# DamRsn/VocoderProject

Measured on AMD Instinct MI355X. Metric: STFT-geometry frames/sec (1024-pt frames, hop 256) through the pitch-corrector/vocoder path, higher is better.
Workload: dtype f64

## Files before the change

### vocoderproject_amd/csrc/vp_common.h

```cpp
#pragma once
#include <stddef.h>

#define VP_MARKS 64
#define VP_ORDER_MAX 100
#define VP_ORDER_MAX_SYNTH 30
#define VP_NOTES_STRIDE 89

struct VpGeom {
    int S, N, F, H, C, cpf, W, h, toKeep, latency, inSize, outSize, tauMax;
    int eLen;
    int orderPitch;
    int tau0;
    int bufferIdxMax;
    int xsSteps;
    int htabGlobal;
    double fs, delta, yinTol;
    double gateThrSum;
    double levEps;
    double eeFloor;
};

struct VpCall {
    int inCounter, outCounter, currCounter;
    int vStart, nWin;
// ... 54 lines not shown
    unsigned int *fault;
    int spinLimit;
    const int *streamMap;
};

#if defined(__HIPCC__)
#define VP_HD __host__ __device__
#else
#define VP_HD
#endif

VP_HD static inline int vp_dy_len(int tauMax) { const int need = 2 * VP_MARKS + (5 * VP_MARKS + 1) / 2; return tauMax + 1 > need ? tauMax + 1 : need; }
VP_HD static inline int vp_cum_len(int tauMax) { return tauMax + 1 > 448 ? tauMax + 1 : 448; }

VP_HD static inline size_t vp_pitch_lds_bytes(const VpGeom &g)
{
    size_t dbl = (size_t)(g.toKeep + g.F) + 12 + (size_t)(g.xsSteps - 1) * g.C + g.eLen + 2 * (size_t)g.F + (size_t)vp_dy_len(g.tauMax) + (size_t)vp_cum_len(g.tauMax) + 2 * (VP_ORDER_MAX + 1) + (2 * (size_t)g.tauMax + 4) + (g.htabGlobal ? 0 : 2 * (size_t)g.tauMax + 2);
    return dbl * sizeof(double) + 8 * 16 + sizeof(VpPitchState) + 64 + 64;
}
VP_HD static inline size_t vp_pitch_acc_lds_bytes(const VpGeom &g) { return ((size_t)g.N + g.C + 1 + g.C + 128) * sizeof(double) + 16; }

#define WS_MAXI 24
#define WS_MAXS 8
#define WS_NBG 4
#define WS_ORDER_MAX 24
#define WS_AF(g) ((g).orderPitch > 15 ? 32 : 16)
#define WS_HP(g) ((g).orderPitch > 16 ? 192 : 128)
#define WS_HIST(g) ((g).orderPitch > 15 ? 32 : 16)

struct WsCtl {
    int psDone;
    int fillTurn;
    int bgPub, bgAdopt;
    int prodBar, bgBar;
    int xcDone, zeroDone, pDone, acDone, lpcDone, pickState, pickDone;
    int tDone;
    int pickT[2];
    int iirDone;
    int pubMode;
    int lpcZ[2];
    int instMode[WS_MAXI];
    int ishareBG[4], ishareP[4];
    int fftFlag[4];
    int gNext[WS_MAXS + 1];
    int gDone[WS_MAXI];
    int gNT[WS_MAXS + 1], gLo[WS_MAXS + 1], gHi[WS_MAXS + 1], gNg[WS_MAXS + 1];
};

struct VpWsSched {
    int nInst, nStart, nSeg;
    int instStep[WS_MAXI], instK[WS_MAXI], instPar[WS_MAXI], instStart[WS_MAXI];
    int startStep[WS_MAXS], startPar[WS_MAXS], startNeed[WS_MAXS];
    int segA[WS_MAXS + 1], segB[WS_MAXS + 1];
};
VP_HD static inline bool ws_build_sched(const VpGeom &g, int nChunk0, int nSteps, VpWsSched &sc)
{
    int nCh = nChunk0, par = 0, nI = 0, nS = 0, nG = 0;
    int lastUse[2] = {0, 0};
    for (int t = 0; t < nSteps; t++) {
        if (nCh != 0) {
            if (nI >= WS_MAXI) return false;
            if (nI == 0) { if (nG > WS_MAXS) return false; sc.segA[nG] = 0; sc.segB[nG] = 0; nG++; }
            sc.instStep[nI] = t; sc.instK[nI] = nCh; sc.instPar[nI] = par; sc.instStart[nI] = -1;
            sc.segB[nG - 1] = nI;
            nI++;
            lastUse[par] = nI;
        }
        if (nCh == g.cpf - 1) nCh = 0;
        if (nCh == 0) {
            if (nI >= WS_MAXI || nS >= WS_MAXS || nG > WS_MAXS) return false;
            par ^= 1;
            sc.instStep[nI] = t; sc.instK[nI] = 0; sc.instPar[nI] = par; sc.instStart[nI] = nS;
            sc.startStep[nS] = t; sc.startPar[nS] = par; sc.startNeed[nS] = lastUse[par];
            sc.segA[nG] = nI; sc.segB[nG] = nI; nG++;
            nI++; nS++;
            lastUse[par] = nI;
        }
        nCh += 1;
    }
    sc.nInst = nI; sc.nStart = nS; sc.nSeg = nG;
    return nI > 0;
}

#define WS_MB_MAX 16
#define WS_MB_SCHEDS 4
struct VpWsMb {
    int nBlocks;
    int schedOf[WS_MB_MAX], nChunk0[WS_MB_MAX], inCtr[WS_MB_MAX], outCtr[WS_MB_MAX], currCtr[WS_MB_MAX];
    VpWsSched sc[WS_MB_SCHEDS];
};

struct WsCarve {
    int xs, eF, fr, qtab, htab, P, dY, gtab, r, aPrev, hp, aF, xp, hist, tw, oA, st, ctl, end;
};
VP_HD static inline int ws_even(int v) { return (v + 1) & ~1; }
VP_HD static inline WsCarve ws_carve(const VpGeom &g, int nSteps)
{
    WsCarve c;
    int o = 0;
    c.xs = o;    o += ws_even(g.toKeep + g.F + (nSteps - 1) * g.C + 4);
    c.eF = o;    o += ws_even(g.eLen);
    c.fr = o;    o += 4 * g.F + 2048;
    c.qtab = o;  o += ws_even(2 * g.tauMax + 4);
    c.htab = o;  o += ws_even(2 * g.tauMax + 2);
    c.P = o;     o += ws_even(g.F + g.tauMax + 2 > 450 ? g.F + g.tauMax + 2 : 450);
    c.dY = o;    o += ws_even(vp_dy_len(g.tauMax) + 1);
    c.gtab = o;  o += 2 * VP_MARKS + (6 * VP_MARKS + 1) / 2 + 1;
    o = ws_even(o);
    c.r = o;     o += 2 * 64;
    c.aPrev = o; o += 2 * (VP_ORDER_MAX + 1 + 1);
    c.hp = o;    o += 2 * WS_HP(g);
    c.aF = o;    o += 2 * WS_AF(g);
    c.xp = o;    o += (g.orderPitch > 15 ? 128 : 64);
    c.hist = o;  o += 2 * WS_HIST(g);
    c.tw = o;    o += 2 * VP_FFT_TW_D2;
    c.oA = o;    o += ws_even(g.N + g.C + 1);
    c.st = o;    o += 2 * ((int)(sizeof(VpPitchState) + 15) / 16 * 2);
    c.ctl = o;   o += ((int)sizeof(WsCtl) + 7) / 8;
    c.end = ws_even(o);
    return c;
}
VP_HD static inline size_t vp_pitch_ws_lds_bytes(const VpGeom &g, int nSteps) { return (size_t)ws_carve(g, nSteps).end * sizeof(double); }

VP_HD static inline size_t voc_wave_doubles(int W)
{
    return (size_t)4 * W + 2 * (VP_ORDER_MAX + 1) + 2 * (VP_ORDER_MAX_SYNTH + 1) + 2;
}
#define VP_VOC_SHARED_DOUBLES(W) ((size_t)(W) + 20 + 16 + 8)
```

### vocoderproject_amd/csrc/vp_filters.inc

```

__device__ __forceinline__ double bcast_f64(double v, int src)
{
    int lo = __double2loint(v), hi = __double2hiint(v);
    lo = __builtin_amdgcn_readlane(lo, src);
    hi = __builtin_amdgcn_readlane(hi, src);
    return __hiloint2double(hi, lo);
}

template <class RP, class AP>
__device__ __forceinline__ bool levinson_wave(RP r, AP a, int order, int aLen, double eps, lds_f64 *scratch = nullptr)
{
    const int lane = vp_tid() & 63;
    if (fabs(r[0]) < eps) {
        for (int i = lane; i < aLen; i += WAVE) a[i] = (i == 0) ? 1.0 : 0.0;
        return true;
    }
    const double r0 = r[0];
    if (scratch && order < WAVE) {
        typedef double d2 __attribute__((ext_vector_type(2)));
        typedef __attribute__((address_space(3))) d2 lds_d2;
        lds_d2 *pr = (lds_d2 *)scratch;
        double av = 0.0;
        if (lane == 0) av = 1.0;
        if (lane == 1) av = r[1] / r0;
// ... 840 lines not shown
#define VP_BI_ROW(XQ, Q) \
    VP_BI_T(acc0, XQ, H[16 * Q + 0], 0);   VP_BI_T(acc1, XQ, H[16 * Q + 1], 1);   VP_BI_T(acc2, XQ, H[16 * Q + 2], 2);   \
    VP_BI_T(acc3, XQ, H[16 * Q + 3], 3);   VP_BI_T(acc0, XQ, H[16 * Q + 4], 4);   VP_BI_T(acc1, XQ, H[16 * Q + 5], 5);   \
    VP_BI_T(acc2, XQ, H[16 * Q + 6], 6);   VP_BI_T(acc3, XQ, H[16 * Q + 7], 7);   VP_BI_T(acc0, XQ, H[16 * Q + 8], 8);   \
    VP_BI_T(acc1, XQ, H[16 * Q + 9], 9);   VP_BI_T(acc2, XQ, H[16 * Q + 10], 10); VP_BI_T(acc3, XQ, H[16 * Q + 11], 11); \
    VP_BI_T(acc0, XQ, H[16 * Q + 12], 12); VP_BI_T(acc1, XQ, H[16 * Q + 13], 13); VP_BI_T(acc2, XQ, H[16 * Q + 14], 14); \
    VP_BI_T(acc3, XQ, H[16 * Q + 15], 15);
template <bool RAGGED = false>
__device__ __forceinline__ void iir_block_wave_regs(const lds_f64 *x, lds_f64 *y, int n, const lds_f64 *aL, int order_,
                                                    bool haveHist0, const lds_f64 *hpad)
{
    const int lane = vp_tid() & 63, m = lane & 15;
    const int order = __builtin_amdgcn_readfirstlane(order_);
    {
        double H[64];
#pragma unroll
        for (int j = 16; j < 64; j++) H[j] = hpad[WAVE + lane - j];
        for (int b = 0; b < n; b += WAVE) {
            double X1 = x[RAGGED ? min(b + 16 + m, n - 1) : b + 16 + m], X2 = x[RAGGED ? min(b + 32 + m, n - 1) : b + 32 + m], X3 = x[RAGGED ? min(b + 48 + m, n - 1) : b + 48 + m];
            if (RAGGED) { X1 = (b + 16 + m < n) ? X1 : 0.0; X2 = (b + 32 + m < n) ? X2 : 0.0; X3 = (b + 48 + m < n) ? X3 : 0.0; asm volatile("s_nop 1" : "+v"(X1), "+v"(X2), "+v"(X3)); }
            double acc0 = 0.0, acc1 = 0.0, acc2 = 0.0, acc3 = 0.0;
            VP_BI_ROW(X1, 1)
            VP_BI_ROW(X2, 2)
            VP_BI_ROW(X3, 3)
            if (!RAGGED || b + lane < n) y[b + lane] = (acc0 + acc1) + (acc2 + acc3);
        }
    }
    double H[16], A[16];
#pragma unroll
    for (int j = 0; j < 16; j++) H[j] = hpad[WAVE + lane - j];
#pragma unroll
    for (int k = 1; k <= 16; k++) A[k - 1] = (m + k <= order) ? -aL[m + k] : 0.0;
    double X0 = (!RAGGED || m < n) ? x[RAGGED ? min(m, n - 1) : m] : 0.0;
    for (int b = 0; b < n; b += WAVE) {
        const bool hist = (b > 0) || haveHist0;
        double Y3 = 0.0;
        if (hist && 16 - m <= order) Y3 = y[b - 16 + m];
        const double parked = (!RAGGED || b + lane < n) ? y[RAGGED ? min(b + lane, n - 1) : b + lane] : 0.0;
        double u0 = 0.0, u1 = 0.0;
        VP_BI_T(u0, Y3, A[0], 15);  VP_BI_T(u1, Y3, A[1], 14);  VP_BI_T(u0, Y3, A[2], 13);  VP_BI_T(u1, Y3, A[3], 12);
        VP_BI_T(u0, Y3, A[4], 11);  VP_BI_T(u1, Y3, A[5], 10);  VP_BI_T(u0, Y3, A[6], 9);   VP_BI_T(u1, Y3, A[7], 8);
        VP_BI_T(u0, Y3, A[8], 7);   VP_BI_T(u1, Y3, A[9], 6);   VP_BI_T(u0, Y3, A[10], 5);  VP_BI_T(u1, Y3, A[11], 4);
        VP_BI_T(u0, Y3, A[12], 3);  VP_BI_T(u1, Y3, A[13], 2);  VP_BI_T(u0, Y3, A[14], 1);  VP_BI_T(u1, Y3, A[15], 0);
        X0 = X0 + (u0 + u1);
        asm volatile("s_nop 1" : "+v"(X0));
        double acc0 = 0.0, acc1 = 0.0, acc2 = 0.0, acc3 = 0.0;
        VP_BI_ROW(X0, 0)
        if (!RAGGED || b + lane < n) y[b + lane] = parked + ((acc0 + acc1) + (acc2 + acc3));
        const int bn = b + WAVE;
        if (bn < n) X0 = (!RAGGED || bn + m < n) ? x[RAGGED ? min(bn + m, n - 1) : bn + m] : 0.0;
    }
}

__device__ __forceinline__ void iir_hc_phase1(const lds_f64 *x, lds_f64 *y, int n, const lds_f64 *hpad, double gmul)
{
    const int lane = vp_tid() & 63, m = lane & 15;
    {
        double H[64];
#pragma unroll
        for (int j = 0; j < 64; j++) H[j] = hpad[WAVE + lane - j];
        for (int b = 0; b < n; b += WAVE) {
            double X0 = gmul * x[b + m], X1 = gmul * x[b + 16 + m], X2 = gmul * x[b + 32 + m], X3 = gmul * x[b + 48 + m];
            double acc0 = 0.0, acc1 = 0.0, acc2 = 0.0, acc3 = 0.0;
            asm volatile("s_nop 1" : "+v"(X0), "+v"(X1), "+v"(X2), "+v"(X3));
            VP_BI_ROW(X0, 0)
            VP_BI_ROW(X1, 1)
            VP_BI_ROW(X2, 2)
            VP_BI_ROW(X3, 3)
            y[b + lane] = (acc0 + acc1) + (acc2 + acc3);
        }
    }
}
template <int RN = 48>
__device__ __forceinline__ void iir_hc_phase2(lds_f64 *y, int n, const lds_f64 *aL, int order_, int nh0, const lds_f64 *hpad,
                                              int *flag = nullptr, int gen = 0, const VpTmo *timeouts = nullptr)
{
    static_assert(RN == 32 || RN == 48, "32 or 48 history columns");
    const int lane = vp_tid() & 63, m = lane & 15;
    const int order = __builtin_amdgcn_readfirstlane(order_);
    STAMPG_BEGIN();
    double R[RN];
    {
        const lds_f64 *h = hpad + WAVE;
        const double h0 = h[lane + 1], h1 = (lane + 65 < 128) ? h[lane + 65] : 0.0;
        double c0 = h0, c1 = h1;
        R[0] = c0;
        const double areg = (lane + 1 <= order) ? aL[lane + 1] : 0.0;
#pragma unroll
        for (int k = 1; k < RN; k++) {
            const double ak = bcast_f64(areg, k - 1);
            const double up = bcast_f64(c1, 0);
            double n0 = wave_shl1_f64(c0);
            const double n1 = wave_shl1_f64(c1);
            if (lane == 63) n0 = up;
            c0 = __builtin_fma(ak, h0, n0);
            c1 = __builtin_fma(ak, h1, n1);
            R[k] = c0;
        }
    }
    STAMPG(24);
    if (flag) {
        int spin = 0;
        const int lim = timeouts ? timeouts->limit : (1 << 22);
        for (; spin < lim && __hip_atomic_load(flag, __ATOMIC_ACQUIRE, __HIP_MEMORY_SCOPE_WORKGROUP) != gen; spin++)
            __builtin_amdgcn_s_sleep(1);
        if (spin == lim && lane == 0 && timeouts) vp_timeout(*timeouts);
// ... 92 lines not shown
```

### vocoderproject_amd/csrc/vp_pitch_ws.inc

```

#ifdef VP_STAMPS
#define WS_SLOT(D, W, E) (D).dbg[64 + g.S + (c.nChunk0 & 3) * 128 + (W) * 8 + (E)]
#define WS_EV(D, W, E) do { if (blockIdx.x == 0 && (threadIdx.x & 63) == 0) atomicAdd(&WS_SLOT(D, W, E), (unsigned long long)wall_clock64()); } while (0)
#define WS_EV0(D, W, E) do { if (blockIdx.x == 0 && threadIdx.x == 0) atomicAdd(&WS_SLOT(D, W, E), (unsigned long long)wall_clock64()); } while (0)
#define WS_TB() unsigned long long ws_tb_ = wall_clock64()
#define WS_TA(D, W, E) do { if (blockIdx.x == 0 && (threadIdx.x & 63) == 0) { const unsigned long long t_ = wall_clock64(); atomicAdd(&WS_SLOT(D, W, E), t_ - ws_tb_); ws_tb_ = t_; } } while (0)
#define WS_TR() do { ws_tb_ = wall_clock64(); } while (0)
#define WS_FINE(D, K) do { if (i == 0) WS_EV(D, 12 + (K) / 8, (K) % 8); } while (0)
#define WS_FINEP(D, K) do { if (si == 0 && rank < 2) WS_EV(D, 13 + rank, K); } while (0)
#define WS_FINER(D, J) do { if ((J) < 7) WS_EV(D, 15, J); } while (0)
#define WS_STAT(D, K, V) do { if (blockIdx.x == 0 && (threadIdx.x & 63) == 0) atomicAdd(&(D).dbg[64 + g.S + (K)], (unsigned long long)(V)); } while (0)
#define WS_CLK() wall_clock64()
#else
#define WS_EV(D, W, E) do { } while (0)
#define WS_EV0(D, W, E) do { } while (0)
#define WS_TB() do { } while (0)
#define WS_TA(D, W, E) do { } while (0)
#define WS_TR() do { } while (0)
#define WS_FINE(D, K) do { } while (0)
#define WS_FINEP(D, K) do { } while (0)
#define WS_FINER(D, J) do { } while (0)
#define WS_STAT(D, K, V) do { } while (0)
#define WS_CLK() 0ULL
#endif
// ... 30 lines not shown
    double loc = 0.0;
#pragma unroll
    for (int u = 0; u < 24; u++) { const int j = j0 + u; if (u < per && j < nb) loc += v[u] * v[u]; }
    double inc = loc;
    for (int off = 1; off < WAVE; off <<= 1) { const double o = __shfl_up(inc, off, WAVE); if (lane >= off) inc += o; }
    double run = inc - loc;
#pragma unroll
    for (int u = 0; u < 24; u++) { const int j = j0 + u; if (u < per && j <= nb) { P[j] = run; if (j < nb) run += v[u] * v[u]; } }
}

__device__ __forceinline__ void ws_yin_pick_wave(const VpGeom &g, const VpDev &d, const PitchLds &L, lds_state *st)
{
    const int lane = vp_tid() & 63;
    for (int k = 1 + lane; k < g.tauMax; k += WAVE) {
        const double cm = L.cum[k], q = (double)k / cm;
        L.dY[k] = L.dY[k] * q;
    }
    wave_sync();
    int tau = INT_MAX;
    for (int k0 = g.tau0; k0 < g.tauMax; k0 += WAVE) {
        const int k = k0 + lane;
        const unsigned long long m = __ballot(k < g.tauMax && L.dY[min(k, g.tauMax - 1)] < g.yinTol);
        if (m) { tau = k0 + (int)__builtin_ctzll(m); break; }
    }
    if (tau < g.tauMax) {
        while (true) {
            const double a = L.dY[tau + 1], b = L.dY[tau];
            if (!(a < b)) break;
            tau += 1;
            if (tau + 1 >= g.tauMax) break;
        }
        if (lane == 0) {
            if (tau >= g.tauMax) atomicAdd(&d.ub[3], 1ULL);
            st->pitch = g.fs / tau;
            st->period = tau;
        }
    }
}


struct SegTab {
    lds_f64 *x0, *xN;
    lds_i32 *stMark, *srcBase, *flags, *startIdx, *stopIdx, *eLim;
};
__device__ __forceinline__ SegTab ws_seg_tab(lds_f64 *base)
{
    SegTab G;
    G.x0 = base; G.xN = base + VP_MARKS;
    G.stMark = (lds_i32 *)(base + 2 * VP_MARKS); G.srcBase = G.stMark + VP_MARKS; G.flags = G.srcBase + VP_MARKS;
    G.startIdx = G.flags + VP_MARKS; G.stopIdx = G.startIdx + VP_MARKS; G.eLim = G.stopIdx + VP_MARKS;
    return G;
}
__device__ __forceinline__ void ws_psola_table_seg(const VpGeom &g, const VpDev &d, const lds_state *st, lds_state *stIdx, const SegTab &G, int kFirst, int kLast,
                                                   int pSFirst, lds_ctl *ctl, int sg)
{
    const int lane = vp_tid() & 63;
    const int T = (st->pitch > 1) ? st->period : st->prevVoicedPeriod;
    const int nG = 2 * T + 1;
    const int nSt = st->nSt;
    const int smi0 = stIdx->stMarkIdx;
    const int smi = smi0 + lane;
    const bool have = smi < nSt;
    const int stMark = have ? st->stMarks[smi] : 0;
    const int v = stMark - T;
    const int kd = max(kFirst, v >= 0 ? v / g.C : 0);
    const bool due = have && kd <= kLast;
    const unsigned long long notDue = ~__ballot(due);
    const int ng = notDue ? (int)__builtin_ctzll(notDue) : 64;
    if (lane < ng) {
        const int pS = pSFirst + (kd - kFirst) * g.C;
        bool q2 = false;
        int clIdx = closest_an_mark_idx(g, st, stMark, T, kd, pS, q2);
        if (q2) atomicAdd(&d.ub[0], 1ULL);
        int clAnMark;
        if (clIdx >= 0)
            clAnMark = st->anMarks[clIdx];
        else {
            int j = st->nPrevAn - clIdx;
            atomicAdd(&d.ub[1], 1ULL);
            clAnMark = (j >= 0 && j < VP_MARKS) ? st->prevAnMarks[j] : 0;
        }
        const double dSt = (double)stMark;
        const double beta = st->beta;
        const double x0 = dSt + (double)(0 - T) / beta;
        const double xN = dSt + (double)(nG - 1 - T) / beta;
        G.x0[lane] = x0; G.xN[lane] = xN;
        G.stMark[lane] = stMark;
        G.srcBase[lane] = g.toKeep + clAnMark - T;
        G.flags[lane] = (smi == 0 ? 1 : 0) | (smi == nSt - 1 ? 2 : 0);
        G.startIdx[lane] = max(max((int)floor(x0), 0), kd * g.C);
        G.stopIdx[lane] = min((int)ceil(xN), g.F);
        G.eLim[lane] = min(g.eLen, g.toKeep + g.F + kd * g.C);
    }
    int lo = 0, hi = 0;
    if (lane < ng) { lo = G.startIdx[lane]; hi = G.stopIdx[lane]; }
    lo = __builtin_amdgcn_readfirstlane(lo);
#pragma unroll
    for (int off = 32; off > 0; off >>= 1) hi = max(hi, __shfl_xor(hi, off, WAVE));
    if (lane == 0) {
        stIdx->stMarkIdx = smi0 + ng;
        ctl->gNg[sg] = ng; ctl->gLo[sg] = lo; ctl->gHi[sg] = hi;
        ctl->gNT[sg] = (ng > 0 && hi > lo) ? (hi - lo + WAVE - 1) / WAVE : 0;
    }
}
__device__ __forceinline__ void ws_psola_gather_seg(const VpGeom &g, const VpDev &d, const PitchLds &L, const SegTab &G, lds_ctl *ctl, int sg, int jA, int jB,
                                                    int kFirst, bool first)
{
    const lds_state *st = L.st;
    const int lane = vp_tid() & 63;
    const int nT = ctl->gNT[sg], lo = ctl->gLo[sg], hi = ctl->gHi[sg], ng = ctl->gNg[sg];
    const lds_f64 *hw = L.htab;
    bool have = false;
    int T = 0, nG = 1;
    double beta = 1.0, mx0 = 0.0, mxN = 0.0;
    int mst = 0, msrc = 0, mfl = 0, ma = 0, mb = 0, mlim = 0;
    auto below = [&](int x) -> int { return (x <= lo) ? 0 : min((x - lo + WAVE - 1) / WAVE, nT); };
    auto count = [&](int r) -> int {
        const int a = (r == 0) ? 0 : below((kFirst + r) * g.C), b = (r == jB - jA) ? nT : below((kFirst + r + 1) * g.C);
        return b - a;
    };
    auto release = [&](int j) {
        ws_wait_ge(&ctl->psDone, j, d);
        for (;;) {
            if (lane == 0) ctl->instMode[j] = 2;
            ws_signal(&ctl->psDone, j + 1);
            j++;
            if (j > jB || count(j - jA) != 0) break;
        }
    };
    if (first) {
        if (count(0) == 0) release(jA);
    }
    for (;;) {
        int m = 0;
        if (lane == 0) m = __hip_atomic_fetch_add((lds_i32 *)&ctl->gNext[sg], 1, __ATOMIC_RELAXED, __HIP_MEMORY_SCOPE_WORKGROUP);
        m = __builtin_amdgcn_readfirstlane(m);
        if (m >= nT) break;
        const unsigned long long tTrip0 = WS_CLK();
        (void)tTrip0;
        if (!have) {
            have = true;
            T = (st->pitch > 1) ? st->period : st->prevVoicedPeriod;
            nG = 2 * T + 1;
            beta = st->beta;
            const int ql = max(min(lane, ng - 1), 0);
            mx0 = G.x0[ql]; mxN = G.xN[ql];
            mst = G.stMark[ql]; msrc = G.srcBase[ql]; mfl = G.flags[ql]; ma = G.startIdx[ql]; mb = G.stopIdx[ql]; mlim = G.eLim[ql];
        }
        const int b = lo + WAVE * m;
        const int i = b + lane;
        const bool in = i < hi;
        const double di = (double)i;
        double accv = in ? L.oE[i] : 0.0;
        unsigned long long mask = __ballot(lane < ng && ma < b + WAVE && mb > b);
        struct Entry { int sa, sb, stM, srcBase, fl, eLim; double x0, xN; };
        auto entry = [&](int q) -> Entry {
            Entry e;
            e.sa = __builtin_amdgcn_readlane(ma, q); e.sb = __builtin_amdgcn_readlane(mb, q);
            e.x0 = __hiloint2double(__builtin_amdgcn_readlane(__double2hiint(mx0), q), __builtin_amdgcn_readlane(__double2loint(mx0), q));
            e.xN = __hiloint2double(__builtin_amdgcn_readlane(__double2hiint(mxN), q), __builtin_amdgcn_readlane(__double2loint(mxN), q));
            e.stM = __builtin_amdgcn_readlane(mst, q); e.srcBase = __builtin_amdgcn_readlane(msrc, q); e.fl = __builtin_amdgcn_readlane(mfl, q);
            e.eLim = __builtin_amdgcn_readlane(mlim, q);
            return e;
        };
        auto slow = [&](const Entry &e, bool &act) -> double {
            act = in && i >= e.sa && i < e.sb && di >= e.x0 && di <= e.xN;
            if (!act) return 0.0;
            const double dSt = (double)e.stM;
            int j = (int)ceil((di - dSt) * beta) + T;
            j = max(0, min(j, nG - 1));
            const double q0 = L.qtab[j], qm = L.qtab[max(j - 1, 0)], qp = L.qtab[min(j + 1, nG - 1)];
            double xj = dSt + q0, xjm = 0.0;
            if (j < nG - 1 && xj < di) {
                xjm = xj; j++; xj = dSt + qp;
                while (j < nG - 1 && xj < di) { xjm = xj; j++; xj = dSt + L.qtab[j]; }
            } else if (j > 0) {
                xjm = dSt + qm;
// ... 9 lines not shown
                const int src = e.srcBase + jj;
                const double ev = (src >= 0 && src < e.eLim) ? L.eF[src] : 0.0;
                const bool windowed = (e.fl & 1) ? (jj >= T) : ((e.fl & 2) ? (jj < T) : true);
                return windowed ? ev * hw[jj] : ev;
            };
            if (j > 0) {
                const double ya = ys(j - 1), yb = ys(j);
                return ya + (yb - ya) / (xj - xjm) * (di - xjm);
            }
            return ys(0);
        };
        auto fast = [&](const Entry &e, bool &act, bool &ok) -> double {
            act = in && i >= e.sa && i < e.sb && di >= e.x0 && di <= e.xN;
            const double dSt = (double)e.stM;
            int j0 = (int)ceil((di - dSt) * beta) + T;
            j0 = max(0, min(j0, nG - 1));
            const double q0 = L.qtab[j0], qm = L.qtab[max(j0 - 1, 0)], qp = L.qtab[min(j0 + 1, nG - 1)];
            const double xj0 = dSt + q0, xm0 = dSt + qm, xp0 = dSt + qp;
            const bool up = j0 < nG - 1 && xj0 < di;
            const bool upMore = up && (j0 + 1 < nG - 1) && xp0 < di;
            const bool down = !up && j0 > 0 && xm0 >= di;
            ok = !act || !(upMore || down);
            const int j = up ? j0 + 1 : j0;
            const double xj = up ? xp0 : xj0, xjm = up ? xj0 : xm0;
            const int ja = max(j - 1, 0);
            const int srcA = e.srcBase + ja, srcB = e.srcBase + j;
            const double ea = L.eF[max(0, min(srcA, e.eLim - 1))], eb = L.eF[max(0, min(srcB, e.eLim - 1))];
            const double ha = hw[ja], hb = hw[j];
            const double eva = (srcA >= 0 && srcA < e.eLim) ? ea : 0.0, evb = (srcB >= 0 && srcB < e.eLim) ? eb : 0.0;
            const bool wa = (e.fl & 1) ? (ja >= T) : ((e.fl & 2) ? (ja < T) : true), wb = (e.fl & 1) ? (j >= T) : ((e.fl & 2) ? (j < T) : true);
            const double ya = wa ? eva * ha : eva, yb = wb ? evb * hb : evb;
            const double itp = ya + (yb - ya) / (xj - xjm) * (di - xjm);
            return (j > 0) ? itp : yb;
        };
        while (mask) {
            const int q1 = (int)__builtin_ctzll(mask);
            mask &= mask - 1;
            const bool two = mask != 0;
            const int q2 = two ? (int)__builtin_ctzll(mask) : q1;
            mask &= mask - 1;
            const Entry e1 = entry(q1), e2 = entry(q2);
            bool a1, a2, ok1, ok2;
            double v1 = fast(e1, a1, ok1), v2 = fast(e2, a2, ok2);
            WS_STAT(d, 2, 1);
#ifdef WS_GATHER_TEST
            if (WS_GATHER_TEST == 1) ok1 = false;
            if (WS_GATHER_TEST == 2 && ((b >> 6) & 1) && lane == 5) ok2 = false;
#endif
            if (__ballot(!(ok1 && ok2))) { v1 = slow(e1, a1); v2 = slow(e2, a2); WS_STAT(d, 3, 1); }
            if (a1) accv += v1;
            if (two && a2) accv += v2;
        }
        if (in) L.oE[i] = accv;
        WS_STAT(d, 0, 1); WS_STAT(d, 1, WS_CLK() - tTrip0);
        int r = 0;
        for (int q = 1; q <= jB - jA; q++) r += (b >= (kFirst + q) * g.C) ? 1 : 0;
        __threadfence_block();
        int was = 0;
        if (lane == 0) was = __hip_atomic_fetch_add((lds_i32 *)&ctl->gDone[jA + r], 1, __ATOMIC_ACQ_REL, __HIP_MEMORY_SCOPE_WORKGROUP);
        was = __builtin_amdgcn_readfirstlane(was);
        if (was + 1 == count(r)) release(jA + r);
    }
}

template <bool FAST, bool BIG>
__device__ __forceinline__ void ws_background(const VpGeom &g0, const VpCall &c, const VpDev &d, const VpWsSched &sc, lds_f64 *sm, const WsCarve &cv0,
                                              lds_ctl *ctl, int bw, int gateOpen)
{
    lds_state *stBG = (lds_state *)(sm + cv0.st) + 1;
    const bool lead = bw == WS_NBG - 1;
    int bgBarGen = 0;
    PitchLds L;
    L.qtab = nullptr; L.htab = nullptr;
    L.st = stBG;
    L.ishare = (int *)ctl->ishareBG;
    L.fftFlag = (int *)ctl->fftFlag;
    L.xcA = nullptr;
    L.oA = nullptr; L.pend = nullptr;
    L.gateOpen = gateOpen;
    const int wq = (int)(blockDim.x / WAVE) - WS_NBG + bw;
    (void)wq;
    const int nStart = sc.nStart;
    for (int i = 0; i < nStart; i++) {
        const int gen = i + 1;
        VpGeom g = g0;
        WsCarve cv = cv0;
        asm volatile("" : "+s"(g.tauMax), "+s"(g.F), "+s"(g.C), "+s"(g.toKeep), "+s"(g.orderPitch), "+s"(g.tau0));
        asm volatile("" : "+s"(cv.xs), "+s"(cv.fr), "+s"(cv.P), "+s"(cv.dY), "+s"(cv.r), "+s"(cv.aPrev), "+s"(cv.hp), "+s"(cv.xp), "+s"(cv.aF), "+s"(cv.tw));
        L.eF = sm + cv.P;
        L.cum = sm + cv.P;
        L.dY = sm + cv.dY;
        L.fftTw = (lds_d2 *)(sm + cv.tw);
        if (lead) WS_FINE(d, 0);
        const int lane = vp_tid() & 63;
        if (!gateOpen) {
            if (lead) {
                ws_wait_ge(&ctl->bgAdopt, i, d);
                if (lane == 0) { stBG->nAn = 0; stBG->prevPitch = 0; stBG->gateOpen = 0; ctl->pubMode = 0; }
                ws_signal(&ctl->bgPub, gen);
            }
            continue;
        }
        const int pn = sc.startPar[i], tS = sc.startStep[i];
        ws_wait_ge(&ctl->fillTurn, sc.startNeed[i], d);
        if (i == 0) WS_EV(d, wq, 0);
        L.xs = sm + cv.xs + ((g.toKeep - g.tauMax) & 1) + tS * g.C;
// ... 122 lines not shown
            WS_FINE(d, 2);
            pitch_marks(g, L, d.ub);
            WS_FINE(d, 3);
            place_st_marks(g, c, d, stBG, nr, notesN);
        }
        wave_sync();
        if (i == 0) WS_EV(d, wq, 4);
        ws_wait_ge(&ctl->lpcDone, gen, d);
        if (stBG->nAn != 0) {
            const int ncopy = ctl->lpcZ[pn] ? VP_ORDER_MAX + 1 : g.orderPitch + 1;
            for (int q = lane; q < ncopy; q += WAVE) stBG->a[q] = L.aPrev[q];
        }
        WS_FINE(d, 4);
        ws_wait_ge(&ctl->zeroDone, (WS_NBG - 1) * gen, d);
        WS_FINE(d, 5);
        if (lane == 0) ctl->pubMode = stBG->nAn != 0 ? 2 : 1;
        ws_signal(&ctl->bgPub, gen);
        WS_EV(d, wq, i == 0 ? 5 : 6);
        VP_PRIO_DOWN();
    }
}

template <bool FAST>
__device__ __forceinline__ void ws_producer(const VpGeom &g, const VpCall &c, const VpDev &d, const VpWsSched &sc, lds_f64 *sm, const WsCarve &cv,
                                            lds_ctl *ctl, int rank, int nP, int gateOpen, bool firstBlock = true, bool lastBlock = true)
{
    const int lane = vp_tid() & 63, tp = rank * WAVE + lane, ntp = nP * WAVE;
    lds_state *st = (lds_state *)(sm + cv.st), *stPub = st + 1;
    lds_f64 *xsAll = sm + cv.xs + ((g.toKeep - g.tauMax) & 1);
    lds_f64 *frBase = sm + cv.fr;
    int barGen = 0;
    bool qValid = false;
    PitchLds L;
    L.st = st;
    L.eF = sm + cv.eF;
    L.qtab = sm + cv.qtab;
    L.htab = sm + cv.htab;
    const SegTab G = ws_seg_tab(sm + cv.gtab);
    const int order = g.orderPitch;
    const int wq = rank + 2;
    (void)wq;
    WS_EV(d, wq, 0);
    WS_TB();
    const int s_ = vp_stream(d);
    if (firstBlock && c.nChunk0 != 0 && st->nAn != 0) {
        const double *ge = d.eFrame + (size_t)s_ * g.eLen;
        const int lim = min(g.eLen, g.toKeep + g.F + (c.nChunk0 - 1) * g.C);
        for (int q = tp; q < lim; q += ntp) L.eF[q] = ge[q];
    }
    for (int sg = 0; sg < sc.nSeg; sg++) {
        const int jA = sc.segA[sg], jB = sc.segB[sg];
        const int t = sc.instStep[jA], kFirst = sc.instK[jA], kLast = sc.instK[jB], p = sc.instPar[jA], si = sc.instStart[jA];
        const int pS = c.pStart + t * g.C;
        WS_TR();
        L.xs = xsAll + t * g.C;
        L.oE = p ? frBase + 3 * g.F + 2048 : frBase;
        L.yF = p ? frBase + 2 * g.F + 2048 : frBase + g.F;
        int mode;
        if (si >= 0) {
            const int jEnd = g.toKeep + g.F + (jB - jA) * g.C;
            if (gateOpen && rank != 0) {
                ws_wait_ge(&ctl->lpcDone, si + 1, d);
                WS_TA(d, wq, 1);
                const lds_f64 *aN = sm + cv.aF + p * WS_AF(g);
                for (int q = 4 * (tp - WAVE); q < jEnd; q += 4 * (ntp - WAVE)) fir4((const lds_f64 *)L.xs, aN, order, q, jEnd, L.eF);
                for (int q = jEnd + tp - WAVE; q < g.eLen; q += ntp - WAVE) L.eF[q] = 0.0;
                WS_TA(d, wq, 2);
                ws_wait_ge(&ctl->tDone, si + 1, d);
                WS_TA(d, wq, 1);
                const int T = ctl->pickT[p];
                const double *hg = d.hannTab + d.hannOff[T];
                for (int q = tp - WAVE; q < 2 * T + 1; q += ntp - WAVE) L.htab[q] = hg[q];
                WS_TA(d, wq, 2);
            }
            ws_wait_ge(&ctl->bgPub, si + 1, d);
            WS_TA(d, wq, 1);
            WS_FINEP(d, 0);
            mode = ctl->pubMode;
            if (rank == 0) {
                if (mode == 2) {
                    if (lane == 0) st->stMarkIdx = 0;
                    wave_sync();
                    ws_psola_table_seg(g, d, stPub, st, G, kFirst, kLast, pS, ctl, sg);
                }
                WS_TA(d, wq, 4);
                WS_FINEP(d, 2);
            } else {
                if (rank == 1) {
                    const int keep = (int)(offsetof(VpPitchState, stMarkIdx) / sizeof(int));
                    const lds_i32 *src = (const lds_i32 *)stPub;
                    lds_i32 *dst = (lds_i32 *)st;
                    for (int q = lane; q < (int)(sizeof(VpPitchState) / sizeof(int)); q += WAVE) if (q != keep) dst[q] = src[q];
                    WS_FINEP(d, 1);
                }
                if (mode == 2) {
                    const int T = (stPub->pitch > 1) ? stPub->period : stPub->prevVoicedPeriod;
                    const double beta = stPub->beta;
                    for (int q = tp - WAVE; q < 2 * T + 1; q += ntp - WAVE) L.qtab[q] = (double)(q - T) / beta;
                }
                WS_TA(d, wq, 2);
                WS_FINEP(d, 2);
            }
            if (mode == 1) for (int q = tp; q < jEnd; q += ntp) L.eF[q] = 0.0;
            qValid = mode == 2;
            ws_group_barrier(&ctl->prodBar, nP, barGen, d);
            WS_TA(d, wq, 3);
            WS_FINEP(d, 3);
            if (rank == 0) ws_signal(&ctl->bgAdopt, si + 1);
        } else {
            mode = (st->nAn != 0) ? 2 : 0;
            if (mode == 2) {
                if (rank == 0) {
                    ws_psola_table_seg(g, d, st, st, G, kFirst, kLast, pS, ctl, sg);
                    WS_TA(d, wq, 4);
                } else {
                    const int j0 = g.toKeep + g.F - g.C, jEnd = j0 + (jB - jA + 1) * g.C;
                    for (int q = j0 + 4 * (tp - WAVE); q < jEnd; q += 4 * (ntp - WAVE)) fir4((const lds_f64 *)L.xs, (const lds_f64 *)st->a, order, q, jEnd, L.eF + kFirst * g.C);
                    for (int q = kFirst * g.C + jEnd + tp - WAVE; q < g.eLen; q += ntp - WAVE) L.eF[q] = 0.0;
                    if (!qValid) {
                        const int T = (st->pitch > 1) ? st->period : st->prevVoicedPeriod;
                        const double beta = st->beta;
                        const double *hg = d.hannTab + d.hannOff[T];
                        for (int q = tp - WAVE; q < 2 * T + 1; q += ntp - WAVE) { L.qtab[q] = (double)(q - T) / beta; L.htab[q] = hg[q]; }
                    }
                    WS_TA(d, wq, 2);
                }
                qValid = true;
                ws_group_barrier(&ctl->prodBar, nP, barGen, d);
                WS_TA(d, wq, 3);
            }
        }
        if (mode == 2) {
            ws_psola_gather_seg(g, d, L, G, ctl, sg, jA, jB, kFirst, rank == 0);
            WS_FINEP(d, 4);
            WS_TA(d, wq, 5);
            ws_wait_ge(&ctl->psDone, jB + 1, d);
            WS_FINEP(d, 6);
            WS_TA(d, wq, 3);
        } else {
            ws_group_barrier(&ctl->prodBar, nP, barGen, d);
            WS_TA(d, wq, 3);
            if (rank == 0) {
                if (lane <= jB - jA) ctl->instMode[jA + lane] = (lane == 0) ? mode : 0;
                ws_signal(&ctl->psDone, jB + 1);
            }
        }
    }
    {
        int nChunkEnd = c.nChunk0;
        for (int t = 0; t < c.nSteps; t++) { if (nChunkEnd == g.cpf - 1) nChunkEnd = 0; nChunkEnd += 1; }
        if (lastBlock && nChunkEnd != 0 && st->nAn != 0) {
            double *ge = d.eFrame + (size_t)s_ * g.eLen;
            for (int q = tp; q < g.eLen; q += ntp) ge[q] = L.eF[q];
        }
    }
    WS_EV(d, wq, 7);
}

template <bool FAST, bool BIG>
__device__ __forceinline__ void ws_recursion(const VpGeom &g, const VpCall &c, const VpDev &d, const VpWsSched &sc, lds_f64 *sm, const WsCarve &cv,
                                             lds_ctl *ctl, int me, int nIir, double gainPitch)
{
    const int nInst = sc.nInst;
    const int lane = vp_tid() & 63;
    lds_f64 *frBase = sm + cv.fr, *oA = sm + cv.oA;
    const int order = g.orderPitch;
    const int nW = g.C / WAVE;
    VP_PRIO_UP();
    WS_EV(d, me, 0);
    WS_TB();
    auto fill = [&](int j, const double (&win)[8]) {
        const int p = sc.instPar[j], pS = c.pStart + sc.instStep[j] * g.C, shift = sc.instK[j] * g.C;
        const lds_f64 *yF = p ? frBase + 2 * g.F + 2048 : frBase + g.F;
        if (ctl->instMode[j] >= 1) {
#pragma unroll
            for (int u = 0; u < 8; u++) if (u < nW) {
                const int i = lane + WAVE * u;
                oA[pS + i] += yF[shift + i] * win[u] * gainPitch;
            }
        }
        ws_signal(&ctl->fillTurn, j + 1);
    };
    auto window = [&](int j, double (&win)[8]) {
        const int shift = sc.instK[j] * g.C;
#pragma unroll
        for (int u = 0; u < 8; u++) win[u] = (u < nW) ? d.pitchStWin[shift + lane + WAVE * u] : 0.0;
    };
    int fj = 0;
    auto flush = [&](int upto, bool block) {
        for (; fj < upto; fj++) {
            if (sc.instPar[fj] != me) continue;
            if (!block && __hip_atomic_load(&ctl->fillTurn, __ATOMIC_ACQUIRE, __HIP_MEMORY_SCOPE_WORKGROUP) < fj) break;
            ws_wait_ge(&ctl->fillTurn, fj, d);
            double win[8];
            window(fj, win);
            fill(fj, win);
        }
    };
    for (int j = 0; j < nInst; j++) {
        const int p = sc.instPar[j];
        if (nIir > 1 && p != me) continue;
        WS_TR();
        const int k = sc.instK[j], shift = k * g.C;
        lds_f64 *oE = p ? frBase + 3 * g.F + 2048 : frBase, *yF = p ? frBase + 2 * g.F + 2048 : frBase + g.F;
        const lds_f64 *aF = sm + cv.aF + p * WS_AF(g), *hpad = sm + cv.hp + p * WS_HP(g);
        if (!FAST && nIir > 1) {
            int spin = 0;
            while (__hip_atomic_load(&ctl->psDone, __ATOMIC_ACQUIRE, __HIP_MEMORY_SCOPE_WORKGROUP) < j + 1) {
                flush(j, false);
                if (++spin >= d.spinLimit) { if (lane == 0) vp_timeout(vp_tmo(d, 61)); break; }
                __builtin_amdgcn_s_sleep(1);
            }
        } else
        ws_wait_ge(&ctl->psDone, j + 1, d);
        WS_TA(d, me, 1);
        if (me == 0) WS_FINER(d, j);
        const int mode = ctl->instMode[j];
        if (mode == 2) {
            if (FAST)
            {
                if (BIG && order > 16) iir_block_wave_hc<32>((const lds_f64 *)(oE + shift), yF + shift, g.C, aF, order, min(order, shift), hpad, 1.0);
                else iir_block_wave_regs((const lds_f64 *)(oE + shift), yF + shift, g.C, aF, order, shift > 0, hpad);
            } else {
                lds_f64 *hist = sm + cv.hist + me * WS_HIST(g);
                const int nh = min(order, shift);
                for (int q = 0; q < order; q++) hist[q] = (q < nh) ? yF[shift - 1 - q] : 0.0;
                if (BIG && order > 16) iir_exact_lane<24>((const lds_f64 *)(oE + shift), yF + shift, g.C, aF, order, (const lds_f64 *)hist, 1.0);
                else iir_exact_row16((const lds_f64 *)(oE + shift), yF + shift, g.C, aF, order, (const lds_f64 *)hist, 1.0);
            }
        }
        WS_TA(d, me, 2);
        if (FAST)
            ws_signal(&ctl->iirDone, j + 1);
        else
            flush(j + 1, false);
        WS_TA(d, me, 4);
    }
    if (!FAST) { WS_TR(); flush(nInst, true); WS_TA(d, me, 3); }
    WS_EV(d, me, me == 0 ? 6 : 7);
    VP_PRIO_DOWN();
}

__device__ __forceinline__ void ws_filler(const VpGeom &g, const VpCall &c, const VpDev &d, const VpWsSched &sc, lds_f64 *sm, const WsCarve &cv,
                                          lds_ctl *ctl, double gainPitch)
{
    const int lane = vp_tid() & 63;
    lds_f64 *frBase = sm + cv.fr, *oA = sm + cv.oA;
    const int nW = g.C / WAVE;
    VP_PRIO_UP();
    for (int j = 0; j < sc.nInst; j++) {
        const int p = sc.instPar[j], pS = c.pStart + sc.instStep[j] * g.C, shift = sc.instK[j] * g.C;
        const lds_f64 *yF = p ? frBase + 2 * g.F + 2048 : frBase + g.F;
        double win[8];
#pragma unroll
        for (int u = 0; u < 8; u++) win[u] = (u < nW) ? d.pitchStWin[shift + lane + WAVE * u] : 0.0;
        ws_wait_ge(&ctl->iirDone, j + 1, d);
        if (ctl->instMode[j] >= 1) {
#pragma unroll
            for (int u = 0; u < 8; u++) if (u < nW) {
                const int i = lane + WAVE * u;
                oA[pS + i] += yF[shift + i] * win[u] * gainPitch;
            }
        }
        ws_signal(&ctl->fillTurn, j + 1);
    }
    VP_PRIO_DOWN();
}

__device__ __forceinline__ void ws_emit_block(const VpGeom &g, const VpCall &c, const VpDev &d, float *__restrict__ out, const lds_state *stl,
                                              const lds_f64 *oA)
{
    const int s = vp_stream(d);
    const float *vr = d.voiceRing + (size_t)s * g.inSize;
    const float *sr0 = d.synthRing + (size_t)s * 2 * g.inSize;
    const float *sr1 = sr0 + g.inSize;
    double *acc = d.outAcc + (size_t)s * g.outSize;
    double *acc2 = d.outAcc2 ? d.outAcc2 + (size_t)s * g.outSize : nullptr;
    float *o = out + (size_t)s * (c.inplace ? 3 : 2) * g.N;
    const int dryOn = stl->sp.dryOn, synthOn = stl->sp.synthOn;
    const double gainVoice = stl->sp.gainVoice, gainSynth = stl->sp.gainSynth;
    for (int i = vp_tid(); i < g.N; i += blockDim.x) {
        int pos = c.outCounter + i, pin = c.currCounter + i;
        pos -= (pos >= g.outSize) ? g.outSize : 0;
        pin -= (pin >= g.inSize) ? g.inSize : 0;
        double v = oA[i];
        if (acc2) { v += acc2[pos]; acc2[pos] = 0.0; }
        if (dryOn) v += (double)vr[pin] * gainVoice;
        double l = v, r = v;
        if (synthOn) { l += (double)sr0[pin] * gainSynth; r += (double)sr1[pin] * gainSynth; }
// ... 208 lines not shown
```

Before: 24.57 million.

## Park block-IIR partial sums in PSOLA gather for last segment, finish with walk

For the final schedule segment in the fast low-order path, the PSOLA gather wave now computes the history-independent part of the block IIR (the X1..X3 rows) right after producing each output block and stores it in yF. The IIR wave then runs a lighter walk kernel that adds only the recursive history term on top of the parked value, with coefficient registers loaded once per segment. The aim is to move IIR work off the serial critical path into the gather stage. In exchange the table ranges are widened for parked segments, a new instMode value is introduced, and the gather wave carries extra register pressure.

```diff
diff --git a/vocoderproject_amd/csrc/vp_common.h b/vocoderproject_amd/csrc/vp_common.h
--- a/vocoderproject_amd/csrc/vp_common.h
+++ b/vocoderproject_amd/csrc/vp_common.h
@@ -130,6 +130,7 @@
     int instStep[WS_MAXI], instK[WS_MAXI], instPar[WS_MAXI], instStart[WS_MAXI];
     int startStep[WS_MAXS], startPar[WS_MAXS], startNeed[WS_MAXS];
     int segA[WS_MAXS + 1], segB[WS_MAXS + 1];
+    int segPark[WS_MAXS + 1];
 };
 VP_HD static inline bool ws_build_sched(const VpGeom &g, int nChunk0, int nSteps, VpWsSched &sc)
 {
@@ -157,6 +158,13 @@
         nCh += 1;
     }
     sc.nInst = nI; sc.nStart = nS; sc.nSeg = nG;
+    for (int q = 0; q <= WS_MAXS; q++) {
+#ifdef WS_PARK_EVERY
+        sc.segPark[q] = (q < nG) ? 1 : 0;
+#else
+        sc.segPark[q] = (nS > 0 && q == nG - 1) ? 1 : 0;
+#endif
+    }
     return nI > 0;
 }
 
diff --git a/vocoderproject_amd/csrc/vp_filters.inc b/vocoderproject_amd/csrc/vp_filters.inc
--- a/vocoderproject_amd/csrc/vp_filters.inc
+++ b/vocoderproject_amd/csrc/vp_filters.inc
@@ -916,6 +916,60 @@
     }
 }
 
+__device__ __forceinline__ void iir_block_park(const lds_f64 *x, lds_f64 *y, int b, const lds_f64 *hpad)
+{
+    const int lane = vp_tid() & 63, m = lane & 15;
+    double H[64];
+#pragma unroll
+    for (int j = 16; j < 48; j++) H[j] = hpad[WAVE + lane - j];
+    const double X1 = x[b + 16 + m], X2 = x[b + 32 + m], X3 = x[b + 48 + m];
+    double acc0 = 0.0, acc1 = 0.0, acc2 = 0.0, acc3 = 0.0;
+    VP_BI_ROW(X1, 1)
+    asm volatile("" ::: "memory");
+#pragma unroll
+    for (int j = 48; j < 64; j++) H[j] = hpad[WAVE + lane - j];
+    VP_BI_ROW(X2, 2)
+    VP_BI_ROW(X3, 3)
+    y[b + lane] = (acc0 + acc1) + (acc2 + acc3);
+}
+struct IirWalkRegs { double H[16], A[16]; };
+__device__ __forceinline__ void iir_block_walk_load(IirWalkRegs &R, const lds_f64 *aL, int order_, const lds_f64 *hpad)
+{
+    const int lane = vp_tid() & 63, m = lane & 15;
+    const int order = __builtin_amdgcn_readfirstlane(order_);
+#pragma unroll
+    for (int j = 0; j < 16; j++) R.H[j] = hpad[WAVE + lane - j];
+#pragma unroll
+    for (int k = 1; k <= 16; k++) R.A[k - 1] = (m + k <= order) ? -aL[m + k] : 0.0;
+}
+__device__ __forceinline__ void iir_block_walk(const IirWalkRegs &R, const lds_f64 *x, lds_f64 *y, int n, int order_, bool haveHist0)
+{
+    const int lane = vp_tid() & 63, m = lane & 15;
+    const int order = __builtin_amdgcn_readfirstlane(order_);
+    double H[16], A[16];
+#pragma unroll
+    for (int j = 0; j < 16; j++) { H[j] = R.H[j]; A[j] = R.A[j]; }
+    double X0 = x[m];
+    for (int b = 0; b < n; b += WAVE) {
+        const bool hist = (b > 0) || haveHist0;
+        double Y3 = 0.0;
+        if (hist && 16 - m <= order) Y3 = y[b - 16 + m];
+        const double parked = y[b + lane];
+        double u0 = 0.0, u1 = 0.0;
+        VP_BI_T(u0, Y3, A[0], 15);  VP_BI_T(u1, Y3, A[1], 14);  VP_BI_T(u0, Y3, A[2], 13);  VP_BI_T(u1, Y3, A[3], 12);
+        VP_BI_T(u0, Y3, A[4], 11);  VP_BI_T(u1, Y3, A[5], 10);  VP_BI_T(u0, Y3, A[6], 9);   VP_BI_T(u1, Y3, A[7], 8);
+        VP_BI_T(u0, Y3, A[8], 7);   VP_BI_T(u1, Y3, A[9], 6);   VP_BI_T(u0, Y3, A[10], 5);  VP_BI_T(u1, Y3, A[11], 4);
+        VP_BI_T(u0, Y3, A[12], 3);  VP_BI_T(u1, Y3, A[13], 2);  VP_BI_T(u0, Y3, A[14], 1);  VP_BI_T(u1, Y3, A[15], 0);
+        X0 = X0 + (u0 + u1);
+        asm volatile("s_nop 1" : "+v"(X0));
+        double acc0 = 0.0, acc1 = 0.0, acc2 = 0.0, acc3 = 0.0;
+        VP_BI_ROW(X0, 0)
+        y[b + lane] = parked + ((acc0 + acc1) + (acc2 + acc3));
+        const int bn = b + WAVE;
+        if (bn < n) X0 = x[bn + m];
+    }
+}
+
 __device__ __forceinline__ void iir_hc_phase1(const lds_f64 *x, lds_f64 *y, int n, const lds_f64 *hpad, double gmul)
 {
     const int lane = vp_tid() & 63, m = lane & 15;
diff --git a/vocoderproject_amd/csrc/vp_pitch_ws.inc b/vocoderproject_amd/csrc/vp_pitch_ws.inc
--- a/vocoderproject_amd/csrc/vp_pitch_ws.inc
+++ b/vocoderproject_amd/csrc/vp_pitch_ws.inc
@@ -106,7 +106,7 @@
     return G;
 }
 __device__ __forceinline__ void ws_psola_table_seg(const VpGeom &g, const VpDev &d, const lds_state *st, lds_state *stIdx, const SegTab &G, int kFirst, int kLast,
-                                                   int pSFirst, lds_ctl *ctl, int sg)
+                                                   int pSFirst, lds_ctl *ctl, int sg, bool park)
 {
     const int lane = vp_tid() & 63;
     const int T = (st->pitch > 1) ? st->period : st->prevVoicedPeriod;
@@ -151,14 +151,15 @@
     lo = __builtin_amdgcn_readfirstlane(lo);
 #pragma unroll
     for (int off = 32; off > 0; off >>= 1) hi = max(hi, __shfl_xor(hi, off, WAVE));
+    if (park) { lo = kFirst * g.C; hi = max(hi, (kLast + 1) * g.C); }
     if (lane == 0) {
         stIdx->stMarkIdx = smi0 + ng;
         ctl->gNg[sg] = ng; ctl->gLo[sg] = lo; ctl->gHi[sg] = hi;
-        ctl->gNT[sg] = (ng > 0 && hi > lo) ? (hi - lo + WAVE - 1) / WAVE : 0;
+        ctl->gNT[sg] = ((ng > 0 || park) && hi > lo) ? (hi - lo + WAVE - 1) / WAVE : 0;
     }
 }
 __device__ __forceinline__ void ws_psola_gather_seg(const VpGeom &g, const VpDev &d, const PitchLds &L, const SegTab &G, lds_ctl *ctl, int sg, int jA, int jB,
-                                                    int kFirst, bool first)
+                                                    int kFirst, bool first, const lds_f64 *hpPark = nullptr, int nChunk0 = 0)
 {
     const lds_state *st = L.st;
     const int lane = vp_tid() & 63;
@@ -176,7 +177,7 @@
     auto release = [&](int j) {
         ws_wait_ge(&ctl->psDone, j, d);
         for (;;) {
-            if (lane == 0) ctl->instMode[j] = 2;
+            if (lane == 0) ctl->instMode[j] = hpPark ? 3 : 2;
             ws_signal(&ctl->psDone, j + 1);
             j++;
             if (j > jB || count(j - jA) != 0) break;
@@ -292,6 +293,12 @@
             if (two && a2) accv += v2;
         }
         if (in) L.oE[i] = accv;
+        if (hpPark && b < (kFirst + jB - jA + 1) * g.C) {
+            iir_block_park((const lds_f64 *)L.oE, L.yF, b, hpPark);
+#ifdef VP_STAMPS
+            { const struct { int nChunk0; } c = {nChunk0}; if (m == 0) WS_EV(d, 13, 7); }
+#endif
+        }
         WS_STAT(d, 0, 1); WS_STAT(d, 1, WS_CLK() - tTrip0);
         int r = 0;
         for (int q = 1; q <= jB - jA; q++) r += (b >= (kFirst + q) * g.C) ? 1 : 0;
@@ -520,6 +527,8 @@
         const int jA = sc.segA[sg], jB = sc.segB[sg];
         const int t = sc.instStep[jA], kFirst = sc.instK[jA], kLast = sc.instK[jB], p = sc.instPar[jA], si = sc.instStart[jA];
         const int pS = c.pStart + t * g.C;
+        const bool park = FAST && order <= 16 && sc.segPark[sg] != 0;
+        const lds_f64 *hpPark = park ? (const lds_f64 *)(sm + cv.hp + p * WS_HP(g)) : (const lds_f64 *)nullptr;
         WS_TR();
         L.xs = xsAll + t * g.C;
         L.oE = p ? frBase + 3 * g.F + 2048 : frBase;
@@ -549,7 +558,7 @@
                 if (mode == 2) {
                     if (lane == 0) st->stMarkIdx = 0;
                     wave_sync();
-                    ws_psola_table_seg(g, d, stPub, st, G, kFirst, kLast, pS, ctl, sg);
+                    ws_psola_table_seg(g, d, stPub, st, G, kFirst, kLast, pS, ctl, sg, park);
                 }
                 WS_TA(d, wq, 4);
                 WS_FINEP(d, 2);
@@ -579,7 +588,7 @@
             mode = (st->nAn != 0) ? 2 : 0;
             if (mode == 2) {
                 if (rank == 0) {
-                    ws_psola_table_seg(g, d, st, st, G, kFirst, kLast, pS, ctl, sg);
+                    ws_psola_table_seg(g, d, st, st, G, kFirst, kLast, pS, ctl, sg, park);
                     WS_TA(d, wq, 4);
                 } else {
                     const int j0 = g.toKeep + g.F - g.C, jEnd = j0 + (jB - jA + 1) * g.C;
@@ -599,7 +608,7 @@
             }
         }
         if (mode == 2) {
-            ws_psola_gather_seg(g, d, L, G, ctl, sg, jA, jB, kFirst, rank == 0);
+            ws_psola_gather_seg(g, d, L, G, ctl, sg, jA, jB, kFirst, rank == 0, hpPark, c.nChunk0);
             WS_FINEP(d, 4);
             WS_TA(d, wq, 5);
             ws_wait_ge(&ctl->psDone, jB + 1, d);
@@ -665,7 +674,9 @@
             fill(fj, win);
         }
     };
-    for (int j = 0; j < nInst; j++) {
+    int jPark = nInst;
+    if (FAST && order <= 16) for (int sg = sc.nSeg - 1; sg >= 0 && sc.segPark[sg] != 0; sg--) jPark = sc.segA[sg];
+    for (int j = 0; j < jPark; j++) {
         const int p = sc.instPar[j];
         if (nIir > 1 && p != me) continue;
         WS_TR();
@@ -703,6 +714,30 @@
         else
             flush(j + 1, false);
         WS_TA(d, me, 4);
+    }
+    if constexpr (FAST) {
+        IirWalkRegs R;
+        bool haveR = false;
+        for (int j = jPark; j < nInst; j++) {
+            const int p = sc.instPar[j];
+            WS_TR();
+            const int k = sc.instK[j], shift = k * g.C;
+            lds_f64 *oE = p ? frBase + 3 * g.F + 2048 : frBase, *yF = p ? frBase + 2 * g.F + 2048 : frBase + g.F;
+            const lds_f64 *aF = sm + cv.aF + p * WS_AF(g), *hpad = sm + cv.hp + p * WS_HP(g);
+            if (sc.instStart[j] >= 0) haveR = false;
+            else if (!haveR) { iir_block_walk_load(R, aF, order, hpad); haveR = true; }
+            ws_wait_ge(&ctl->psDone, j + 1, d);
+            WS_TA(d, me, 1);
+            WS_FINER(d, j);
+            if (ctl->instMode[j] == 3) {
+                if (!haveR) { iir_block_walk_load(R, aF, order, hpad); haveR = true; }
+                if (j == jPark) WS_EV(d, 14, 7);
+                iir_block_walk(R, (const lds_f64 *)(oE + shift), yF + shift, g.C, order, shift > 0);
+            }
+            WS_TA(d, me, 2);
+            ws_signal(&ctl->iirDone, j + 1);
+            WS_TA(d, me, 4);
+        }
     }
     if (!FAST) { WS_TR(); flush(nInst, true); WS_TA(d, me, 3); }
     WS_EV(d, me, me == 0 ? 6 : 7);
```

Measured after the change: 25.37 million, median of 6. 1.03x the previous value.
